# Meng-333/SRADSGAN

Measured on AMD Instinct MI355X. Metric: training images/sec (216x216, x4), higher is better.
Workload: dtype f32 (split-bf16 products: 3 bf16 MFMA terms per fp32 multiply, fp32 accumulate)

## Files before the change

include/sradsgan_hip.h:

```cpp
#ifndef SRADSGAN_HIP_H
#define SRADSGAN_HIP_H
#include <stddef.h>
#include <stdint.h>

#ifdef __cplusplus
extern "C" {
#endif

#define SRHIP_OK 0
#define SRHIP_ERR_ARG (-1)
#define SRHIP_ERR_LAUNCH (-2)
#define SRHIP_ERR_WORKSPACE (-3)

#define SRHIP_EPI_BIAS 1
#define SRHIP_EPI_LRELU 2
#define SRHIP_EPI_RESIDUAL 4
#define SRHIP_EPI_ROWSCALE 8
#define SRHIP_EPI_ACTMASK 32
#define SRHIP_EPI_CHANSCALE 16
#define SRHIP_EPI_GRADDATA 64

const char* srhip_last_error(void);
int srhip_abi_version(void);
int srhip_stream_fork(void* from_stream, void* to_stream);
// ... 197 lines not shown
int srhip_dp_init(const void* id_in, int rank, int world);
int srhip_dp_world(void);
int srhip_dp_rank(void);
int srhip_dp_allreduce_bucket(float* buf, size_t count, void* stream);
int srhip_dp_broadcast(float* buf, size_t count, int root, void* stream);
int srhip_dp_finalize(void);

size_t srhip_bn_workspace(long rows, int c);
int srhip_bn_train_fwd(const float* x, const float* gamma, const float* beta, float* running_mean,
                       float* running_var, float* y, float* save_mean, float* save_invstd, void* workspace,
                       size_t workspace_bytes, long rows, int c, float eps, float momentum, float slope, int apply_act,
                       void* stream);
int srhip_bn_train_bwd(const float* dy, const float* x, const float* y, const float* gamma, const float* save_mean,
                       const float* save_invstd, float* dx, float* dgamma, float* dbeta, void* workspace,
                       size_t workspace_bytes, long rows, int c, float slope, int apply_act, void* stream);
int srhip_bn_train_bwd_acc(const float* dy, const float* x, const float* y, const float* gamma, const float* save_mean,
                           const float* save_invstd, float* dx, float* dgamma, float* dbeta, float* acc_gamma,
                           float* acc_beta, void* workspace, size_t workspace_bytes, long rows, int c, float slope,
                           int apply_act, void* stream);
int srhip_bn_train_bwd_acc_x(const float* dy, const float* x, const float* gamma, const float* beta, const float* save_mean,
                             const float* save_invstd, float* dx, float* dgamma, float* dbeta, float* acc_gamma,
                             float* acc_beta, void* workspace, size_t workspace_bytes, long rows, int c, float slope,
                             int apply_act, void* stream);
int srhip_bn_train_bwd_acc_xa(const float* dy, const float* x, const float* gamma, const float* beta, const float* save_mean,
                              const float* save_invstd, const float* addend, float* dx, float* dgamma, float* dbeta, float* acc_gamma,
                              float* acc_beta, void* workspace, size_t workspace_bytes, long rows, int c, float slope,
                              int apply_act, void* stream);
int srhip_bn_eval_fwd(const float* x, const float* gamma, const float* beta, const float* running_mean,
                      const float* running_var, float* y, long rows, int c, float eps, float slope, int apply_act,
                      void* stream);
// ... 36 lines not shown
```

sradsgan_amd/_hip.py:

```python
import ctypes
import os

_HERE = os.path.dirname(os.path.abspath(__file__))
LIB_PATH = os.path.join(_HERE, 'lib', 'libsradsgan_hip.so')

_vp, _i, _f, _l, _sz = ctypes.c_void_p, ctypes.c_int, ctypes.c_float, ctypes.c_long, ctypes.c_size_t

SIGNATURES = {
    'srhip_last_error': (ctypes.c_char_p, []),
    'srhip_abi_version': (_i, []),
    'srhip_stream_fork': (_i, [_vp, _vp]),
    'srhip_debug_set': (_i, [_i, _i]),
    'srhip_probe_config': (_i, [_i] * 7),
    'srhip_probe_read': (_i, [_vp, _vp, _i]),
    'srhip_set_conv_math': (_i, [_i]),
    'srhip_get_conv_math': (_i, []),
    'srhip_resample_ksize': (_i, [_i, _i, _i]),
    'srhip_resample_coeffs': (_i, [_i, _i, _i, _vp, _vp]),
    'srhip_resample_pass_u8': (_i, [_vp, _vp, _vp, _vp, _i, _i, _i, _i, _i, _i, _i, _vp]),
    'srhip_u8_to_float': (_i, [_vp, _vp, _l, _vp]),
    'srhip_packed_elems': (_sz, [_i] * 5),
    'srhip_pack_entry_bytes': (_i, []),
    'srhip_packed_is_fast': (_i, [_i] * 5),
    'srhip_pack_weights_batched': (_i, [_vp, _i, _vp]),
# ... 71 lines not shown
    'srhip_mean_bwd': (_i, [_vp] * 2 + [_l, _vp]),
    'srhip_gp_norm_penalty_fwd': (_i, [_vp] * 3 + [_sz, _l, _i, _vp]),
    'srhip_gp_norm_penalty_bwd': (_i, [_vp] * 3 + [_l, _i, _vp]),
    'srhip_bn_eval_fwd': (_i, [_vp] * 6 + [_l, _i, _f, _f, _i, _vp]),
    'srhip_dp_id_bytes': (_i, []),
    'srhip_dp_unique_id': (_i, [_vp]),
    'srhip_dp_init': (_i, [_vp, _i, _i]),
    'srhip_dp_world': (_i, []),
    'srhip_dp_rank': (_i, []),
    'srhip_dp_allreduce_bucket': (_i, [_vp, _sz, _vp]),
    'srhip_dp_broadcast': (_i, [_vp, _sz, _i, _vp]),
    'srhip_dp_finalize': (_i, []),
    'srhip_bn_workspace': (_sz, [_l, _i]),
    'srhip_bn_train_fwd': (_i, [_vp] * 9 + [_sz, _l, _i, _f, _f, _f, _i, _vp]),
    'srhip_bn_train_bwd': (_i, [_vp] * 10 + [_sz, _l, _i, _f, _i, _vp]),
    'srhip_bn_bwd2_workspace': (_sz, [_l, _i]),
    'srhip_bn_train_bwd_bwd': (_i, [_vp] * 11 + [_sz, _l, _i, _f, _i, _vp]),
    'srhip_clam_pool_segments': (_i, []),
    'srhip_clam_pool_max_segments': (_i, []),
    'srhip_clam_pool_partial': (_i, [_vp, _vp, _sz, _i, _i, _i, _i, _vp]),
    'srhip_conv2d_fwd_pool': (_i, [_vp, _vp, _vp, _vp, _vp, _sz, _vp] + [_i] * 8 + [_vp]),
    'srhip_attn_tail_fwd_pooled': (_i, [_vp, _vp, _sz, _i] + [_vp] * 10 + [_i] * 5 + [_vp]),
    'srhip_attn_tail_eval_pooled': (_i, [_vp, _vp, _vp, _sz, _i] + [_vp] * 6 + [_i] * 5 + [_vp]),
    'srhip_sum_n': (_i, [_vp, _i, _vp, _l, _vp]),
    'srhip_ca_segments': (_i, []),
    'srhip_ca_pool_sum': (_i, [_vp, _vp] + [_i] * 3 + [_vp]),
    'srhip_ca_mlp_fwd': (_i, [_vp, _i] + [_vp] * 5 + [_i] * 4 + [_vp]),
    'srhip_ca_scale_res': (_i, [_vp] * 4 + [_i] * 3 + [_vp]),
    'srhip_ca_bwd_partial': (_i, [_vp] * 3 + [_i] * 3 + [_vp]),
    'srhip_ca_mlp_bwd_workspace': (_sz, [_i, _i]),
# ... 61 lines not shown
```

sradsgan_amd/csrc/bn.hip:

```cpp
#include "common.h"

namespace srhip {

__device__ inline float4 f4add(float4 a, float4 b) { return make_float4(a.x + b.x, a.y + b.y, a.z + b.z, a.w + b.w); }

template <int MODE>
__global__ __launch_bounds__(256) void bn_reduce_stage1(const float* __restrict__ a, const float* __restrict__ x,
                                                        const float* __restrict__ y, const float* __restrict__ mean,
                                                        const float* __restrict__ invstd, float* __restrict__ partial,
                                                        long rows, int c, long rows_per_block, float slope, int act,
                                                        const float* __restrict__ gamma = nullptr, const float* __restrict__ beta = nullptr) {
  __shared__ float4 red0[256], red1[256];
  const int tid = threadIdx.x;
  const int q = c / 4, nrl = 256 / q;
  const int cq = tid % q, rl = tid / q;
  const long r0 = (long)blockIdx.x * rows_per_block;
  const long r1 = r0 + rows_per_block < rows ? r0 + rows_per_block : rows;
  float4 s0 = make_float4(0.f, 0.f, 0.f, 0.f), s1 = s0;
  float4 p0, p1;
  if (MODE == 0) {
    p0 = *reinterpret_cast<const float4*>(x + cq * 4);
  } else {
    p0 = *reinterpret_cast<const float4*>(mean + cq * 4);
    p1 = *reinterpret_cast<const float4*>(invstd + cq * 4);
// ... 75 lines not shown
    const float n = (float)rows;
    const float md = s1 / n;
    float var = s2 / n - md * md;
    var = var > 0.f ? var : 0.f;
    const float mu = x[col] + md;
    mean[col] = mu;
    invstd[col] = rsqrtf(var + eps);
    if (running_mean) {
      running_mean[col] = (1.f - momentum) * running_mean[col] + momentum * mu;
      const float unb = rows > 1 ? var * (n / (n - 1.f)) : var;
      running_var[col] = (1.f - momentum) * running_var[col] + momentum * unb;
    }
  }
}

__global__ void bn_bwd_stage2(const float* __restrict__ partial, float* __restrict__ dgamma, float* __restrict__ dbeta,
                              int nblk, int c, float* __restrict__ acc_gamma, float* __restrict__ acc_beta) {
  __shared__ float r0[16 * BN_SUBS], r1[16 * BN_SUBS];
  const int col = blockIdx.x * 16 + (threadIdx.x & 15), sub = threadIdx.x >> 4;
  float a = 0.f, b = 0.f;
  if (col < c)
    for (int k = sub; k < nblk; k += BN_SUBS) {
      a += partial[(size_t)k * 2 * c + col];
      b += partial[(size_t)k * 2 * c + c + col];
    }
  r0[threadIdx.x] = a;
  r1[threadIdx.x] = b;
  __syncthreads();
  if (sub == 0 && col < c) {
    const int t = threadIdx.x;
// ... 271 lines not shown
  hipStream_t st = as_stream(stream);
  const long nblk = bn_nblk(rows), rpb = (rows + nblk - 1) / nblk;
  float* part = static_cast<float*>(workspace);
  hipLaunchKernelGGL(bn_reduce_stage1<0>, dim3((int)nblk), dim3(256), 0, st, nullptr, x, nullptr, nullptr, nullptr, part,
                     rows, c, rpb, 0.f, 0);
  hipLaunchKernelGGL(bn_stats_stage2, dim3(cdiv(c, 16)), dim3(16 * BN_SUBS), 0, st, part, x, save_mean, save_invstd, running_mean,
                     running_var, (int)nblk, c, rows, eps, momentum);
  const long n4 = rows * c / 4;
  int blocks = (int)((n4 + 255) / 256);
  if (blocks > 256 * 16) blocks = 256 * 16;
  hipLaunchKernelGGL(bn_apply_kernel, dim3(blocks), dim3(256), 0, st, x, save_mean, save_invstd, gamma, beta, y, n4, c,
                     slope, apply_act);
  return check_launch("bn_train_fwd");
}

int srhip_bn_eval_fwd(const float* x, const float* gamma, const float* beta, const float* running_mean,
                      const float* running_var, float* y, long rows, int c, float eps, float slope, int apply_act,
                      void* stream) {
  SRHIP_REQUIRE(x && gamma && beta && running_mean && running_var && y, "bn_eval_fwd: null tensor");
  SRHIP_REQUIRE(rows > 0 && c >= 4 && c % 4 == 0, "bn_eval_fwd: C must be a multiple of 4");
  const long n4 = rows * c / 4;
  int blocks = (int)((n4 + 255) / 256);
  if (blocks > 256 * 16) blocks = 256 * 16;
  hipLaunchKernelGGL(bn_eval_kernel, dim3(blocks), dim3(256), 0, as_stream(stream), x, running_mean, running_var, gamma, beta, y,
                     n4, c, eps, slope, apply_act);
  return check_launch("bn_eval_fwd");
}

int srhip_bn_train_bwd(const float* dy, const float* x, const float* y, const float* gamma, const float* save_mean,
                       const float* save_invstd, float* dx, float* dgamma, float* dbeta, void* workspace,
// ... 109 lines not shown
```

sradsgan_amd/csrc/conv_api.hip:

```cpp
#include "conv_internal.h"
#include "conv_dev.h"

using namespace srhip;

namespace srhip {
struct PackEntry {
  const float* w;
  float* packed;
  int cout, cin, kh, kw, mode, fast;
};
__global__ __launch_bounds__(256) void pack_batched_kernel(const PackEntry* __restrict__ tab) {
  const PackEntry e = tab[blockIdx.y];
  const int khkw = e.kh * e.kw;
  if (e.fast) {
    constexpr int LDS_F = 32 * (16 * 9 + 1);
    __shared__ float tile[LDS_F];
    const long total = (long)e.cout * e.cin * khkw;
    const int RO = e.mode == 0 ? 8 : 32;
    const int CI = e.mode == 0 ? (khkw <= 9 ? 64 : 16) : (khkw <= 9 ? 16 : 4);
    const int ld = CI * khkw + 1;
    const int nci = (e.cin + CI - 1) / CI, nco = (e.cout + RO - 1) / RO;
    const int ndst = e.mode == 0 ? e.cout : e.cin, csrc = e.mode == 0 ? e.cin : e.cout;
    const long ndst16 = ((long)ndst + 15) / 16 * 16;
    float* s0 = e.packed;
// ... 291 lines not shown

int srhip_conv2d_fwd_dual(const float* x, const float* packed, const float* bias, const float* residual, const float* rowscale,
                          const float* chanscale, float* y, void* y_pp, int* served, int n, int h, int w, int cin, int cout, int kh,
                          int kw, int stride, int pad, int ldx, int ldy, int ldr, float slope, int flags, void* stream) {
  SRHIP_REQUIRE(y_pp && served && (((uintptr_t)y_pp) & 15) == 0 && ldy == cout, "conv2d_fwd_dual: 16-byte aligned plane buffer, dense fp32 output");
  g_dst2_req.pp = y_pp;
  g_dst2_req.served = 0;
  const int rc = srhip_conv2d_fwd(x, packed, bias, residual, rowscale, chanscale, y, n, h, w, cin, cout, kh, kw, stride, pad, ldx, ldy, ldr,
                                  slope, flags, stream);
  *served = g_dst2_req.served;
  g_dst2_req.pp = nullptr;
  g_dst2_req.served = 0;
  return rc;
}

int srhip_conv2d_fwd_pool(const float* x, const float* packed, const float* bias, float* y, float* pool, size_t pool_sec_bytes,
                          int* nseg_out, int n, int h, int w, int cin, int cout, int ldx, int ldy, int flags, void* stream) {
  SRHIP_REQUIRE(x && packed && y && pool && nseg_out, "conv2d_fwd_pool: null tensor");
  SRHIP_REQUIRE(cout == 64 && ldy == 64 && n > 0 && h > 0 && w > 0 && cin > 0 && ldx >= cin, "conv2d_fwd_pool: 64 dense destination channels");
  SRHIP_REQUIRE((flags & ~SRHIP_EPI_BIAS) == 0 && (!(flags & SRHIP_EPI_BIAS) || bias), "conv2d_fwd_pool: plain or bias epilogue");
  SRHIP_REQUIRE(pool_sec_bytes % 16 == 0 && pool_sec_bytes < (1u << 30) && (((uintptr_t)pool) & 15) == 0 &&
                    pool_sec_bytes >= (size_t)n * POOL_MAXSEG * 64 * sizeof(float),
                "conv2d_fwd_pool: three 16-byte aligned sections of n * max_segments * 64 floats");
  g_pool_req.out = pool;
  g_pool_req.sec_bytes = (unsigned)pool_sec_bytes;
  g_pool_req.served_nseg = 0;
  const int rc = srhip_conv2d_fwd(x, packed, bias, nullptr, nullptr, nullptr, y, n, h, w, cin, cout, 3, 3, 1, 1, ldx, ldy, 0, 0.f, flags, stream);
  const int served = g_pool_req.served_nseg;
  g_pool_req.out = nullptr;
  g_pool_req.served_nseg = 0;
// ... 266 lines not shown
```

sradsgan_amd/csrc/conv_dev.h:

```cpp
#pragma once
#include "conv_internal.h"

namespace srhip {

typedef unsigned int u32x4 __attribute__((ext_vector_type(4)));
typedef unsigned int u32x2 __attribute__((ext_vector_type(2)));
constexpr int FBK = 16;
constexpr int FLS = FBK + 4;
constexpr unsigned F_OOB = 0x80000000u;

struct FastGeom {
  int N, Hs, Ws, C, lds;
  int OH, OW, M;
  int ss;
  int TH, TW, dh0, dhs, dw0, dws;
  int kh0, khs, kw0, kws, KW;
  int Hd, Wd, dsd, ph, pw, ldd, K;
  int ldw, ldr;
  float slope;
  int flags, accumulate, dst_identity;
  unsigned src_bytes, w_bytes;
  int src_pp = 0, dst_pp = 0, src_guard = 0, dst_guard = 0;
  unsigned src_plane_bytes = 0, dst_plane_bytes = 0;
  void* dst2_pp = nullptr;
  int dst2_guard = 0;
  const float* res2 = nullptr;
  const float* res3 = nullptr;
};
struct ResRequest {
  const float* r2 = nullptr;
  const float* r3 = nullptr;
  int served = 0;
};
extern thread_local ResRequest g_res_req;
struct SignRequest {
  void* words = nullptr;
  size_t bytes = 0;
  int mode = 0;
  int served = 0;
};
extern thread_local SignRequest g_sign_req;
long pp_sign_tiles(int n, int h, int w, int cout);
struct PhaseSet {
// ... 134 lines not shown
```

sradsgan_amd/csrc/conv_fast.hip:

```cpp
#include "conv_dev.h"

namespace srhip {

int g_fast_ablate = 0;



template <int BM, int BN, int WM, int WN, int BK, int MATH = 0>
__global__ __launch_bounds__(WM* WN * 64) void fast_conv_kernel(const float* __restrict__ src,
                                                                 const float* __restrict__ wt,
                                                                 const float* __restrict__ bias,
                                                                 const float* __restrict__ residual,
                                                                 const float* __restrict__ rowscale,
                                                                 const float* __restrict__ chanscale,
                                                                 const float* __restrict__ actmask,
                                                                 float* __restrict__ dst, FastGeom g, int nblk_m,
                                                                 int nblk_n) {
  constexpr int NT = WM * WN * 64;
  constexpr int WTM = BM / WM, WTN = BN / WN;
  constexpr int TM = WTM / 32, TN = WTN / 32;
  constexpr int LS = BK + 4;
  constexpr int QPR = BK / 4;
  constexpr int RPP = NT / QPR;
  constexpr int AR = (BM + RPP - 1) / RPP, BR = (BN + RPP - 1) / RPP;
// ... 581 lines not shown
          const int nimg = mm / OHOW;
          const int rem = mm - nimg * OHOW;
          const int oh = rem / g.OW;
          const int ow = rem - oh * g.OW;
          dpix = ((size_t)nimg * g.Hd + (oh * g.dsd + g.ph)) * g.Wd + (ow * g.dsd + g.pw);
        }
        dpx[j] = (unsigned)dpix;
        if (!okq[j]) nq[j] = 0;
        eo[j] = epi_fetch(dpix, nq[j], flags, g, bias, residual, rowscale, actmask, dst, EPI < 0 && g.accumulate != 0);
      }
#pragma unroll
      for (int j = 0; j < EB; ++j)
        if (okq[j]) epi_finish(vq[j], eo[j], dpx[j], nq[j], flags, g, dst, EPI < 0 && g.accumulate != 0);
    }
    if (t + 1 < TM) asm volatile("s_waitcnt lgkmcnt(0)" ::: "memory");
  }
}


template <int BN, int EPI, int PROD = 0>
__global__ __launch_bounds__(256) __attribute__((amdgpu_waves_per_eu(3))) void conv_patch_kernel(const float* __restrict__ src, const float* __restrict__ wt,
                                                          const float* __restrict__ bias,
                                                          const float* __restrict__ residual,
                                                          const float* __restrict__ actmask, float* __restrict__ dst,
                                                          FastGeom g, PatchGeom pg, int nblk_m, int nblk_n) {
  constexpr int NW = 4, BK = 16;
  constexpr int WTM = 64, WTN = BN / 2;
  constexpr int TM = WTM / 32, TN = WTN / 32;
  constexpr int BPW = BN / 64;
  constexpr int MAXP = 3;
// ... 1595 lines not shown
  }
}

static bool shape_ok(int csrc, int kh, int kw) { return csrc % 16 == 0 && kh * kw <= 32 && kh == kw; }
bool fast_fwd_ok(int cin, int cout, int kh, int kw) { return shape_ok(cin, kh, kw); }
bool fast_dgrad_ok(int cin, int cout, int kh, int kw) { return shape_ok(cout, kh, kw); }
bool fast_wgrad_ok(int cin, int cout, int kh, int kw) { return cin % 16 == 0 && cout % 4 == 0 && kh == kw; }

int fast_pack_weight(const float* w, float* packed, int cout, int cin, int kh, int kw, int mode, hipStream_t st) {
  const long total = (long)cout * cin * kh * kw;
  hipLaunchKernelGGL(fast_pack_kernel, dim3(cdiv(total, 256)), dim3(256), 0, st, w, packed, cout, cin, kh, kw, mode);
  return check_launch("fast_pack_weight");
}

thread_local Dst2Request g_dst2_req;
thread_local ResRequest g_res_req;
thread_local PhaseRequest g_phase_req;
int g_conv_math = 0;
int g_fast_dynlds = 0;
template <int BM, int BN, int WM, int WN, int BK>
static int launch_fast(const float* src, const float* wt, const float* bias, const float* residual,
                       const float* rowscale, const float* chanscale, const float* actmask, float* dst,
                       const FastGeom& g, hipStream_t st) {
  const int nbm = cdiv(g.M, BM), nbn = cdiv(g.K, BN);
  hipLaunchKernelGGL((fast_conv_kernel<BM, BN, WM, WN, BK>), dim3(nbm * nbn), dim3(WM * WN * 64), g_fast_dynlds, st, src, wt, bias,
                     residual, rowscale, chanscale, actmask, dst, g, nbm, nbn);
  return check_launch("fast_conv");
}

__global__ __launch_bounds__(256) void dot_conv_kernel(const float* __restrict__ src, const float* __restrict__ wt,
// ... 221 lines not shown
#undef SRHIP_LK
        }
        SRHIP_LPE(64);
#undef SRHIP_LPE
#undef SRHIP_LP
      }
    }
  }
  if (g_fast_cfg != 20 && (g_fast_cfg < 1 || g_fast_cfg == 23 || g_fast_cfg == 24) && !(g.flags & 0x300) && g.K >= 64 && al16 &&
      (!(eflags & SRHIP_EPI_CHANSCALE) || ((uintptr_t)chanscale & 15) == 0)) {
    const int nbm = cdiv(g.M, 128);
    const bool force = g_fast_cfg == -1 || patch_to_dma;
    const long min_tiles = g_conv_math >= 1 ? 128 : 512;
    const bool wide = g.K >= 128 && ((long)nbm * cdiv(g.K, 128) >= min_tiles || force);
    const long b64 = (long)nbm * cdiv(g.K, 64);
    if (wide || b64 >= min_tiles || force) {
#define SRHIP_LD(BN_, EPI_)                                                                                        \
  do {                                                                                                             \
    const int nbn = cdiv(g.K, BN_);                                                                                \
    if (g.dst2_pp) g_dst2_req.served = 1;                                                                          \
    PhaseSet ps_;                                                                                                  \
    int grid_ = nbm * nbn;                                                                                         \
    if (g_phase_req.active) {                            \
      ps_ = g_phase_req.ps;                                                                                        \
      grid_ = 0;                                                                                                   \
      for (int k_ = 0; k_ < ps_.n; ++k_) {                                                                         \
        ps_.first[k_] = grid_;                                                                                     \
        grid_ += ps_.p[k_].nblk_m * nbn;                                                                           \
      }                                                                                                            \
      ps_.first[ps_.n] = grid_;                                                                                    \
      g_phase_req.launched = 1;                                                                                    \
    }                                                                                                              \
    if (g_conv_math == 1) {                                                                                        \
      hipLaunchKernelGGL((fast_conv_dma_kernel<128, BN_, EPI_, 1>), dim3(grid_), dim3(256), g_fast_dynlds, st,     \
                         src, w16, bias, residual, rowscale, chanscale, actmask, dst, g, nbm,                      \
                         nbn, ps_);                                                                                \
    } else                                                                                                         \
      hipLaunchKernelGGL((fast_conv_dma_kernel<128, BN_, EPI_, 0>), dim3(grid_), dim3(256), g_fast_dynlds, st,     \
                         src, wt, bias, residual, rowscale, chanscale, actmask, dst, g, nbm, nbn, ps_);            \
    return check_launch("fast_conv_dma");                                                                          \
  } while (0)
#define SRHIP_LDE(BN_)                                                  \
  do {                                                                  \
    if (g.accumulate) SRHIP_LD(BN_, -1);                                \
    if (eflags == 0) SRHIP_LD(BN_, 0);                                  \
    if (eflags == SRHIP_EPI_BIAS) SRHIP_LD(BN_, 1);                     \
    if (eflags == (SRHIP_EPI_BIAS | SRHIP_EPI_LRELU)) SRHIP_LD(BN_, 3); \
    if (eflags == SRHIP_EPI_ACTMASK) SRHIP_LD(BN_, 32);                 \
    if (eflags == SRHIP_EPI_RESIDUAL) SRHIP_LD(BN_, 4);                 \
    if (eflags == 29) SRHIP_LD(BN_, 29);  \
    SRHIP_LD(BN_, -1);                                                  \
  } while (0)
      if (prod != 0) {
#define SRHIP_LDH(BN_, MATH_)                                                                                       \
  do {                                                                                                              \
    const int nbn = cdiv(g.K, BN_);                                                                                 \
    hipLaunchKernelGGL((fast_conv_dma_kernel<128, BN_, -1, MATH_>), dim3(nbm * nbn), dim3(256), g_fast_dynlds, st,  \
                       src, w16, bias, residual, rowscale, chanscale, actmask, dst, g, nbm, nbn, PhaseSet());       \
// ... 45 lines not shown
  g.OW = (w + 2 * pad - kw) / stride + 1;
  SRHIP_REQUIRE(g.OH > 0 && g.OW > 0, "conv2d_fwd: empty output");
  const long M = (long)n * g.OH * g.OW;
  SRHIP_REQUIRE(M < (1L << 31), "conv2d_fwd: pixel count overflows int32");
  g.M = (int)M; g.ss = stride;
  g.TH = kh; g.TW = kw; g.dh0 = -pad; g.dhs = 1; g.dw0 = -pad; g.dws = 1;
  g.kh0 = 0; g.khs = 1; g.kw0 = 0; g.kws = 1; g.KW = kw;
  g.Hd = g.OH; g.Wd = g.OW; g.dsd = 1; g.ph = 0; g.pw = 0; g.ldd = ldy; g.K = cout;
  g.ldw = kh * kw * cin; g.ldr = ldr; g.slope = slope; g.flags = flags | g_fast_ablate; g.accumulate = 0; g.dst_identity = 1;
  SRHIP_REQUIRE(bytes_ok((long)n * h * w, ldx, cin, &g.src_bytes), "conv2d_fwd: source tensor >= 2 GiB");
  g.w_bytes = (unsigned)((long)cout * g.ldw * 4);
  if (g_dst2_req.pp != nullptr && stride == 1 && cout % 8 == 0 && g.OH == g.Hd && g.OW == g.Wd) {
    g.dst2_pp = g_dst2_req.pp;
    g.dst2_guard = pp_guard(g.Wd);
  }
  return run_fast(x, packed, bias, residual, rowscale, chanscale, nullptr, y, g, st);
}

int fast_conv2d_fwd_pp(const void* x, int x_pp, const float* packed, const float* bias, void* y, int y_pp, int n, int h, int w, int cin,
                       int cout, int ldx, int ldy, float slope, int flags, hipStream_t st) {
  FastGeom g;
  g.N = n; g.Hs = h; g.Ws = w; g.C = cin; g.lds = x_pp ? cin : ldx;
  g.OH = h; g.OW = w;
  const long M = (long)n * h * w;
  SRHIP_REQUIRE(M < (1L << 31), "conv2d_fwd_pp: pixel count overflows int32");
  g.M = (int)M; g.ss = 1;
  g.TH = 3; g.TW = 3; g.dh0 = -1; g.dhs = 1; g.dw0 = -1; g.dws = 1;
  g.kh0 = 0; g.khs = 1; g.kw0 = 0; g.kws = 1; g.KW = 3;
  g.Hd = h; g.Wd = w; g.dsd = 1; g.ph = 0; g.pw = 0; g.ldd = y_pp ? cout : ldy; g.K = cout;
  g.ldw = 9 * cin; g.ldr = 0; g.slope = slope; g.flags = flags; g.accumulate = 0; g.dst_identity = 1;
// ... 404 lines not shown
```

sradsgan_amd/csrc/elementwise.hip:

```cpp
#include <atomic>
#include <mutex>
#include "conv_internal.h"

#include <string.h>

namespace srhip {

static thread_local char g_err[512] = "";

void set_error(const char* fmt, ...) {
  va_list ap;
  va_start(ap, fmt);
  vsnprintf(g_err, sizeof(g_err), fmt, ap);
  va_end(ap);
}

__global__ void lrelu_bwd_kernel(const float4* __restrict__ dy, const float4* __restrict__ y, float4* __restrict__ dx,
                                 long n4, float slope) {
  long i = (long)blockIdx.x * blockDim.x + threadIdx.x;
  long stride = (long)gridDim.x * blockDim.x;
  for (; i < n4; i += stride) {
    float4 g = dy[i], v = y[i];
    g.x = v.x > 0.f ? g.x : g.x * slope;
    g.y = v.y > 0.f ? g.y : g.y * slope;
// ... 370 lines not shown
  if (vec)
    hipLaunchKernelGGL(colsum_stage1<float4>, dim3((int)nblk), dim3(256), 0, st, dy, (float*)workspace, rows, c, ld, rpb);
  else
    hipLaunchKernelGGL(colsum_stage1<float>, dim3((int)nblk), dim3(256), 0, st, dy, (float*)workspace, rows, c, ld, rpb);
  hipLaunchKernelGGL(colsum_stage2, dim3(cdiv(c, 16)), dim3(256), 0, st, (const float*)workspace, db, (int)nblk, c);
  return check_launch("colsum");
}

}

using namespace srhip;

extern "C" {

const char* srhip_last_error(void) { return g_err; }
int srhip_abi_version(void) { return 13; }

int srhip_stream_fork(void* from_stream, void* to_stream) {
  constexpr int RING = 64;
  static hipEvent_t ring[RING];
  static std::atomic<unsigned> next{0};
  static std::once_flag once;
  static bool created = false;
  if (from_stream == to_stream) return SRHIP_OK;
  std::call_once(once, [&]() {
    created = true;
    for (int i = 0; i < RING; ++i)
      if (hipEventCreateWithFlags(&ring[i], hipEventDisableTiming) != hipSuccess) created = false;
  });
  if (!created) {
    set_error("stream_fork: hipEventCreateWithFlags failed");
// ... 190 lines not shown
```

sradsgan_amd/model/layers.py:

```python
import torch
import torch.nn as nn

from .. import ops


class HipConv2d(nn.Conv2d):

    def __init__(self, *args, **kwargs):
        super().__init__(*args, **kwargs)
        k, s, p, d = self.kernel_size, self.stride, self.padding, self.dilation
        if k[0] != k[1] or s[0] != s[1] or p[0] != p[1] or d != (1, 1) or self.groups != 1:
            raise NotImplementedError('HipConv2d: square kernel/stride/pad, dilation 1, groups 1 only')

    def forward(self, x, act_slope=None, residual=None):
        return ops.conv2d(x, self.weight, self.bias, self.stride[0], self.padding[0], act_slope, residual)


class HipBatchNorm2d(nn.BatchNorm2d):

    def forward(self, x, act_slope=None):
        return ops.batch_norm_act(x, self, act_slope)
```

sradsgan_amd/model/sradsgan.py:

```python
import math

import torch
import torch.nn as nn

from .. import ops
from .base_networks import ChannelAttention, SpatialAttention, _Clam, _Slam
from .layers import HipBatchNorm2d, HipConv2d


class GANLoss(nn.Module):

    def __init__(self, gan_type, real_label_val=1.0, fake_label_val=0.0):
        super().__init__()
        self.gan_type = gan_type.lower()
        self.real_label_val, self.fake_label_val = real_label_val, fake_label_val
        if self.gan_type != 'wgan-gp':
            raise NotImplementedError('GAN type [{:s}] is not found'.format(self.gan_type))

    def forward(self, input, target_is_real):
        m = ops.mean(input)
        return -m if target_is_real else m


class CLAM(_Clam):
# ... 232 lines not shown
            if attention and idx == 6:
                entry[2] = [len(layers), len(layers) + 1]
                layers += [ChannelAttention(256), SpatialAttention()]
            self._blocks.append(tuple(entry))
            cin = cout
        layers.append(HipConv2d(cin, 1, 3, 1, 1))
        self.model = nn.Sequential(*layers)

    def forward(self, img):
        x = ops.nhwc(img)
        m = self.model
        for conv_i, bn_i, extra in self._blocks:
            if bn_i is None:
                x = m[conv_i](x, act_slope=0.2)
            else:
                x = m[bn_i](m[conv_i](x), act_slope=0.2)
            for e in extra:
                x = m[e](x)
        return m[len(m) - 1](x)


class FeatureExtractor(nn.Module):

    _CFG = [(3, 64), 'R', (64, 64), 'R', 'P', (64, 128), 'R', (128, 128), 'R', 'P', (128, 256), 'R']

    def __init__(self):
        super().__init__()
        seq = []
        for item in self._CFG:
            seq.append(HipConv2d(item[0], item[1], 3, 1, 1) if isinstance(item, tuple) else nn.Identity())
        self.feature_extractor = nn.Sequential(*seq)
# ... 23 lines not shown
```

sradsgan_amd/ops.py:

```python
import contextlib
import ctypes
import os
import threading
import weakref

import torch
from torch.autograd import Function

from . import _hip

EPI_BIAS, EPI_LRELU, EPI_RESIDUAL, EPI_ROWSCALE, EPI_CHANSCALE, EPI_GRADDATA = 1, 2, 4, 8, 16, 64
CL = torch.channels_last

class _State:
    skip_param_grads = False
    direct_grads = False
    wgrad_stream = None
    skip_ids = frozenset()
    stop_ids = frozenset()
    capturing = False
    wgrad_group = 1
    pending = None
    held = None
    last_out_pp = None
    carry = None
    carry_expect = None
    carry_token = 0
    wgrad_seq = 0
    ready_pairs = None


_state = _State()


def _skip_param_grads(*params):
    if _state.skip_param_grads:
        return True
    return bool(_state.skip_ids) and any(p is not None and id(p) in _state.skip_ids for p in params)


@contextlib.contextmanager
def backward_scope(skip_params=(), stop_at=()):
    prev = (_state.skip_ids, _state.stop_ids)
    _state.skip_ids = frozenset(id(p) for p in skip_params)
# ... 289 lines not shown
    lib = _hip.lib()
    if out_pp is not None:
        served = ctypes.c_int(0)
        _hip.check(lib.srhip_conv2d_fwd_dual(_p(x), _p(packed_weight(w, 0)), _p(bias), _p(residual), _p(rowscale),
                                             _p(chanscale), _p(y), _p(out_pp.buf), ctypes.byref(served),
                                             n, h, wd, cin, cout, kh, kw, stride, pad, cin, cout, cout,
                                             float(slope or 0.0), flags, _stream()), 'conv2d_fwd_dual')
        if not served.value:
            pp_from_f32(y, out=out_pp)
        return y
    _hip.check(lib.srhip_conv2d_fwd(_p(x), _p(packed_weight(w, 0)), _p(bias), _p(residual), _p(rowscale),
                                    _p(chanscale), _p(y),
                                    n, h, wd, cin, cout, kh, kw, stride, pad, cin, cout, cout,
                                    float(slope or 0.0), flags, _stream()), 'conv2d_fwd')
    return y


_POOL_EPI = os.environ.get('SRHIP_POOL_EPI', '1') == '1'


def pool_epilogue_ok(x, w):
    return (_POOL_EPI and x.is_cuda and get_conv_math() == 'bf16x3' and tuple(w.shape[2:]) == (3, 3) and w.shape[0] == 64
            and w.shape[1] % 32 == 0)


def conv2d_fwd_pool_raw(x, w, bias):
    _require_gpu(x, 'conv2d_fwd_pool')
    x = nhwc(x)
    n, cin, h, wd = x.shape
    cout = w.shape[0]
# ... 619 lines not shown

class _ColSum(Function):
    @staticmethod
    def forward(ctx, dy):
        ctx.shape = dy.shape
        return colsum_raw(dy)

    @staticmethod
    def backward(ctx, g):
        return g.view(1, -1, 1, 1).expand(ctx.shape)


class _ConvFwd(Function):

    @staticmethod
    def forward(ctx, x, w, b, residual, stride, pad, slope, graddata=False):
        if slope is not None and residual is not None:
            raise ValueError('conv2d: fused activation and residual are mutually exclusive')
        y = conv2d_fwd_raw(x, w, b, stride, pad, slope, residual, graddata=graddata)
        ctx.stride, ctx.pad, ctx.slope = stride, pad, slope
        ctx.has_bias, ctx.has_res = b is not None, residual is not None
        ctx.save_for_backward(x, w, y if slope is not None else None, b)
        return y

    @staticmethod
    def backward(ctx, dy):
        x, w, y, b = ctx.saved_tensors
        skip = _skip_param_grads(w)
        need_dx = ctx.needs_input_grad[0] and x.data_ptr() not in _state.stop_ids
        if ctx.slope is not None and not need_dx and not skip and ctx.needs_input_grad[1] and ctx.has_bias and \
                ctx.needs_input_grad[2] and _state.direct_grads and not torch.is_grad_enabled() and _WGRAD_ACT and \
                _wgrad_act_direct(w, b, x, dy, y, ctx.slope, ctx.stride, ctx.pad):
            return None, None, None, None, None, None, None, None
        g = dy if ctx.slope is None else _LReluBwd.apply(dy, y, ctx.slope)
        dx = _ConvDgrad.apply(g, w, tuple(x.shape), ctx.stride, ctx.pad) if need_dx else None
        dw = db = None
        want_b = ctx.has_bias and ctx.needs_input_grad[2] and not skip
        if ctx.needs_input_grad[1] and not skip and _state.direct_grads and not torch.is_grad_enabled():
            dw, db = wgrad_for_params(w, b, x, g, ctx.stride, ctx.pad, want_b)
        elif ctx.needs_input_grad[1] and not skip:
            dw, db = _ConvWgrad.apply(x, g, tuple(w.shape), ctx.stride, ctx.pad, want_b)
        elif want_b:
            db = _ColSum.apply(g)
        dres = _passed_through(dy) if (ctx.has_res and ctx.needs_input_grad[3]) else None
        return dx, dw, db, dres, None, None, None, None


class _ConvDgrad(Function):

    @staticmethod
    def forward(ctx, dy, w, x_shape, stride, pad):
        ctx.stride, ctx.pad, ctx.x_shape = stride, pad, x_shape
        ctx.save_for_backward(dy, w)
        return conv2d_dgrad_raw(dy, w, x_shape, stride, pad)

    @staticmethod
    def backward(ctx, ddx):
        dy, w = ctx.saved_tensors
        skip = _skip_param_grads(w)
        d_dy = _ConvFwd.apply(ddx, w, None, None, ctx.stride, ctx.pad, None, True) if ctx.needs_input_grad[0] else None
# ... 20 lines not shown
    def backward(ctx, ddw, ddb):
        x, dy = ctx.saved_tensors
        d_x = d_dy = None
        if ddw is not None:
            ddw = ddw.contiguous()
            if ctx.needs_input_grad[0]:
                d_x = _ConvDgrad.apply(dy, ddw, tuple(x.shape), ctx.stride, ctx.pad)
            if ctx.needs_input_grad[1]:
                d_dy = _ConvFwd.apply(x, ddw, None, None, ctx.stride, ctx.pad, None, True)
        if ddb is not None and ctx.needs_input_grad[1]:
            e = ddb.view(1, -1, 1, 1).expand(dy.shape)
            d_dy = e if d_dy is None else d_dy + e
        return d_x, d_dy, None, None, None, None


def conv2d(x, weight, bias=None, stride=1, padding=0, act_slope=None, residual=None):
    return _ConvFwd.apply(x, weight, bias, residual, stride, padding, act_slope)


_BUS_SUM = os.environ.get('SRHIP_BUS_SUM', '1') == '1'


class _SumN(Function):

    @staticmethod
    def forward(ctx, tokens, *ts):
        _require_gpu(ts[0], 'sum_n')
        ts = [nhwc(t) for t in ts]
        out = torch.empty_like(ts[0], memory_format=CL)
        tab = (ctypes.c_void_p * len(ts))(*[t.data_ptr() for t in ts])
        _hip.check(_hip.lib().srhip_sum_n(tab, len(ts), _p(out), out.numel(), _stream()), 'sum_n')
        ctx.n, ctx.tokens = len(ts), tokens
# ... 760 lines not shown
            gdy, gx, gg = torch.autograd.grad([o for o, _ in pairs], [dy_, x_, g_], [d for _, d in pairs],
                                              allow_unused=True)
        return gdy, gx, None, gg, None, None, None, None, None, None, None, None


class _BNTrainFwd(Function):
    @staticmethod
    def forward(ctx, x, gamma, beta, running_mean, running_var, eps, momentum, slope):
        _require_gpu(x, 'batch_norm')
        xc = nhwc(x)
        n, c, h, w = x.shape
        rows = n * h * w
        lib = _hip.lib()
        y = torch.empty_like(xc, memory_format=CL)
        mean, invstd = torch.empty_like(gamma), torch.empty_like(gamma)
        ws = torch.empty(lib.srhip_bn_workspace(rows, c) // 4, device=x.device, dtype=torch.float32)
        _hip.check(lib.srhip_bn_train_fwd(_p(xc), _p(gamma.detach().contiguous()), _p(beta.detach().contiguous()),
                                          _p(running_mean), _p(running_var), _p(y), _p(mean), _p(invstd), _p(ws),
                                          ws.numel() * 4, rows, c, float(eps), float(momentum), float(slope or 0.0),
                                          int(slope is not None), _stream()), 'bn_train_fwd')
        ctx.eps, ctx.slope = eps, slope
        ctx.save_for_backward(x, y, gamma, mean, invstd, beta)
        return y

    @staticmethod
    def backward(ctx, dy):
        x, y, gamma, mean, invstd, beta = ctx.saved_tensors
        fold = getattr(_state, 'bn_fold', None)
        held = fold.pop((x.data_ptr(), tuple(x.shape)), None) if (fold and not torch.is_grad_enabled()) else None
        if not torch.is_grad_enabled() and not _skip_param_grads(gamma, beta):
            gg, gb = _grad_slot(gamma), _grad_slot(beta)
            if gg is not None and gb is not None:
                dx, _, _ = _BNTrainBwd.apply(dy, x, y, gamma, mean, invstd, ctx.eps, ctx.slope, gg, gb, beta, held)
                return dx, None, None, None, None, None, None, None
        dx, dgamma, dbeta = _BNTrainBwd.apply(dy, x, y, gamma, mean, invstd, ctx.eps, ctx.slope, None, None, beta, held)
# ... 719 lines not shown
```

Baseline: 665.4.

## Fuse BatchNorm batch-statistics reduction into conv forward epilogue

Adds a conv epilogue variant that computes per-wave, per-channel mean and M2 partials straight from the accumulators and writes them to a slot buffer. A new merge kernel combines these slots Chan-style into mean and invstd and updates the running stats, then the existing apply kernel runs. This skips the separate BN stage-1 reduction pass over the conv output in the discriminator's conv+BN blocks. It costs extra epilogue shuffles and registers in the conv kernel, relies on thread-local handoff state and Python-side pointer/version matching, and the pairwise merge may be slightly less numerically stable.

After: 665.0 (median of 6 runs). Within noise of the previous version (-0.0%).

```diff
diff --git a/include/sradsgan_hip.h b/include/sradsgan_hip.h
--- a/include/sradsgan_hip.h
+++ b/include/sradsgan_hip.h
@@ -235,6 +235,13 @@
 int srhip_bn_train_bwd(const float* dy, const float* x, const float* y, const float* gamma, const float* save_mean,
                        const float* save_invstd, float* dx, float* dgamma, float* dbeta, void* workspace,
                        size_t workspace_bytes, long rows, int c, float slope, int apply_act, void* stream);
+size_t srhip_conv2d_bnstat_bytes(int n, int h, int w, int cout, int kh, int kw, int stride, int pad);
+int srhip_conv2d_fwd_bnstat(const float* x, const float* packed, const float* bias, float* y, float* partial, size_t partial_bytes,
+                            int* nslot_out, int* slot_rows_out, int n, int h, int w, int cin, int cout, int kh, int kw, int stride,
+                            int pad, int flags, void* stream);
+int srhip_bn_train_fwd_merged(const float* partial, int nslot, int slot_rows, const float* x, const float* gamma, const float* beta,
+                              float* running_mean, float* running_var, float* y, float* save_mean, float* save_invstd, long rows, int c,
+                              float eps, float momentum, float slope, int apply_act, void* stream);
 int srhip_bn_train_bwd_acc(const float* dy, const float* x, const float* y, const float* gamma, const float* save_mean,
                            const float* save_invstd, float* dx, float* dgamma, float* dbeta, float* acc_gamma,
                            float* acc_beta, void* workspace, size_t workspace_bytes, long rows, int c, float slope,
diff --git a/sradsgan_amd/_hip.py b/sradsgan_amd/_hip.py
--- a/sradsgan_amd/_hip.py
+++ b/sradsgan_amd/_hip.py
@@ -109,6 +109,9 @@
     'srhip_bn_workspace': (_sz, [_l, _i]),
     'srhip_bn_train_fwd': (_i, [_vp] * 9 + [_sz, _l, _i, _f, _f, _f, _i, _vp]),
     'srhip_bn_train_bwd': (_i, [_vp] * 10 + [_sz, _l, _i, _f, _i, _vp]),
+    'srhip_conv2d_bnstat_bytes': (_sz, [_i] * 8),
+    'srhip_conv2d_fwd_bnstat': (_i, [_vp] * 5 + [_sz, _vp, _vp] + [_i] * 10 + [_vp]),
+    'srhip_bn_train_fwd_merged': (_i, [_vp, _i, _i] + [_vp] * 8 + [_l, _i, _f, _f, _f, _i, _vp]),
     'srhip_bn_bwd2_workspace': (_sz, [_l, _i]),
     'srhip_bn_train_bwd_bwd': (_i, [_vp] * 11 + [_sz, _l, _i, _f, _i, _vp]),
     'srhip_clam_pool_segments': (_i, []),
diff --git a/sradsgan_amd/csrc/bn.hip b/sradsgan_amd/csrc/bn.hip
--- a/sradsgan_amd/csrc/bn.hip
+++ b/sradsgan_amd/csrc/bn.hip
@@ -113,6 +113,54 @@
   }
 }
 
+__global__ void bn_stats_merge(const float* __restrict__ partial, int nslot, int slot_rows, float* __restrict__ mean,
+                               float* __restrict__ invstd, float* __restrict__ running_mean, float* __restrict__ running_var, int c,
+                               long rows, float eps, float momentum) {
+  __shared__ float r0[16 * BN_SUBS], r1[16 * BN_SUBS], r2[16 * BN_SUBS], r3[16 * BN_SUBS];
+  const int col = blockIdx.x * 16 + (threadIdx.x & 15), sub = threadIdx.x >> 4;
+  float s0 = 0.f, s1 = 0.f, s2 = 0.f, sq = 0.f;
+  const float K = col < c ? partial[col] : 0.f;
+  if (col < c) {
+    const long full = rows / slot_rows;
+#pragma unroll 4
+    for (int k = sub; k < nslot; k += BN_SUBS) {
+      const float nb = k < full ? (float)slot_rows : (float)(k == full ? rows - full * slot_rows : 0);
+      const float d = partial[(size_t)k * 2 * c + col] - K;
+      const float q = partial[(size_t)k * 2 * c + c + col];
+      s0 += nb;
+      s1 += nb * d;
+      s2 += nb * d * d;
+      sq += nb > 0.f ? q : 0.f;
+    }
+  }
+  r0[threadIdx.x] = s0;
+  r1[threadIdx.x] = s1;
+  r2[threadIdx.x] = s2;
+  r3[threadIdx.x] = sq;
+  __syncthreads();
+  if (sub == 0 && col < c) {
+    const int t = threadIdx.x;
+    for (int k = 1; k < BN_SUBS; ++k) {
+      s0 += r0[t + 16 * k];
+      s1 += r1[t + 16 * k];
+      s2 += r2[t + 16 * k];
+      sq += r3[t + 16 * k];
+    }
+    const float nr = (float)rows;
+    const float md = s1 / s0;
+    float var = (sq + (s2 - s1 * md)) / nr;
+    var = var > 0.f ? var : 0.f;
+    const float mu = K + md;
+    mean[col] = mu;
+    invstd[col] = rsqrtf(var + eps);
+    if (running_mean) {
+      running_mean[col] = (1.f - momentum) * running_mean[col] + momentum * mu;
+      const float unb = rows > 1 ? var * (nr / (nr - 1.f)) : var;
+      running_var[col] = (1.f - momentum) * running_var[col] + momentum * unb;
+    }
+  }
+}
+
 __global__ void bn_bwd_stage2(const float* __restrict__ partial, float* __restrict__ dgamma, float* __restrict__ dbeta,
                               int nblk, int c, float* __restrict__ acc_gamma, float* __restrict__ acc_beta) {
   __shared__ float r0[16 * BN_SUBS], r1[16 * BN_SUBS];
@@ -414,6 +462,24 @@
   return check_launch("bn_train_fwd");
 }
 
+int srhip_bn_train_fwd_merged(const float* partial, int nslot, int slot_rows, const float* x, const float* gamma, const float* beta,
+                              float* running_mean, float* running_var, float* y, float* save_mean, float* save_invstd, long rows, int c,
+                              float eps, float momentum, float slope, int apply_act, void* stream) {
+  SRHIP_REQUIRE(partial && x && gamma && beta && y && save_mean && save_invstd, "bn_train_fwd_merged: null tensor");
+  SRHIP_REQUIRE(rows > 0 && c >= 4 && c % 4 == 0, "bn_train_fwd_merged: C must be a multiple of 4");
+  SRHIP_REQUIRE(nslot > 0 && slot_rows > 0 && (long)nslot * slot_rows >= rows, "bn_train_fwd_merged: the slots do not cover the rows");
+  SRHIP_REQUIRE((running_mean == nullptr) == (running_var == nullptr), "bn_train_fwd_merged: running stats come in pairs");
+  hipStream_t st = as_stream(stream);
+  hipLaunchKernelGGL(bn_stats_merge, dim3(cdiv(c, 16)), dim3(16 * BN_SUBS), 0, st, partial, nslot, slot_rows, save_mean, save_invstd,
+                     running_mean, running_var, c, rows, eps, momentum);
+  const long n4 = rows * c / 4;
+  int blocks = (int)((n4 + 255) / 256);
+  if (blocks > 256 * 16) blocks = 256 * 16;
+  hipLaunchKernelGGL(bn_apply_kernel, dim3(blocks), dim3(256), 0, st, x, save_mean, save_invstd, gamma, beta, y, n4, c,
+                     slope, apply_act);
+  return check_launch("bn_train_fwd_merged");
+}
+
 int srhip_bn_eval_fwd(const float* x, const float* gamma, const float* beta, const float* running_mean,
                       const float* running_var, float* y, long rows, int c, float eps, float slope, int apply_act,
                       void* stream) {
diff --git a/sradsgan_amd/csrc/conv_api.hip b/sradsgan_amd/csrc/conv_api.hip
--- a/sradsgan_amd/csrc/conv_api.hip
+++ b/sradsgan_amd/csrc/conv_api.hip
@@ -329,6 +329,37 @@
   return rc;
 }
 
+size_t srhip_conv2d_bnstat_bytes(int n, int h, int w, int cout, int kh, int kw, int stride, int pad) {
+  if (n <= 0 || h <= 0 || w <= 0 || cout <= 0 || kh <= 0 || kw <= 0 || stride <= 0 || pad < 0) return 0;
+  const long oh = (h + 2 * pad - kh) / stride + 1, ow = (w + 2 * pad - kw) / stride + 1;
+  if (oh <= 0 || ow <= 0) return 0;
+  const long slots = cdiv(n * oh * ow, 2L * BNSTAT_ROWS) * 2;
+  return (size_t)slots * 2 * cout * sizeof(float);
+}
+int srhip_conv2d_fwd_bnstat(const float* x, const float* packed, const float* bias, float* y, float* partial, size_t partial_bytes,
+                            int* nslot_out, int* slot_rows_out, int n, int h, int w, int cin, int cout, int kh, int kw, int stride,
+                            int pad, int flags, void* stream) {
+  SRHIP_REQUIRE(x && packed && y && partial && nslot_out && slot_rows_out, "conv2d_fwd_bnstat: null tensor");
+  SRHIP_REQUIRE((flags & ~SRHIP_EPI_BIAS) == 0 && (!(flags & SRHIP_EPI_BIAS) || bias), "conv2d_fwd_bnstat: plain or bias epilogue");
+  const size_t need = srhip_conv2d_bnstat_bytes(n, h, w, cout, kh, kw, stride, pad);
+  SRHIP_REQUIRE(need > 0 && partial_bytes >= need && (((uintptr_t)partial) & 15) == 0, "conv2d_fwd_bnstat: partial buffer too small");
+  *nslot_out = 0;
+  *slot_rows_out = BNSTAT_ROWS;
+  const bool fast = fast_fwd_ok(cin, cout, kh, kw);
+  if (fast) {
+    g_bnstat_req.out = partial;
+    g_bnstat_req.served = 0;
+  }
+  const int rc = srhip_conv2d_fwd(x, packed, bias, nullptr, nullptr, nullptr, y, n, h, w, cin, cout, kh, kw, stride, pad, cin, cout, 0, 0.f,
+                                  flags, stream);
+  const int served = fast ? g_bnstat_req.served : 0;
+  g_bnstat_req.out = nullptr;
+  g_bnstat_req.served = 0;
+  if (rc != SRHIP_OK) return rc;
+  if (served) *nslot_out = (int)(need / (2 * cout * sizeof(float)));
+  return SRHIP_OK;
+}
+
 int srhip_conv2d_fwd_pool(const float* x, const float* packed, const float* bias, float* y, float* pool, size_t pool_sec_bytes,
                           int* nseg_out, int n, int h, int w, int cin, int cout, int ldx, int ldy, int flags, void* stream) {
   SRHIP_REQUIRE(x && packed && y && pool && nseg_out, "conv2d_fwd_pool: null tensor");
diff --git a/sradsgan_amd/csrc/conv_dev.h b/sradsgan_amd/csrc/conv_dev.h
--- a/sradsgan_amd/csrc/conv_dev.h
+++ b/sradsgan_amd/csrc/conv_dev.h
@@ -26,7 +26,15 @@
   int dst2_guard = 0;
   const float* res2 = nullptr;
   const float* res3 = nullptr;
+  float* bnstat = nullptr;
 };
+constexpr int BNSTAT_EPI = 0x800;
+constexpr int BNSTAT_ROWS = 64;
+struct BnStatRequest {
+  float* out = nullptr;
+  int served = 0;
+};
+extern thread_local BnStatRequest g_bnstat_req;
 struct ResRequest {
   const float* r2 = nullptr;
   const float* r3 = nullptr;
diff --git a/sradsgan_amd/csrc/conv_fast.hip b/sradsgan_amd/csrc/conv_fast.hip
--- a/sradsgan_amd/csrc/conv_fast.hip
+++ b/sradsgan_amd/csrc/conv_fast.hip
@@ -619,6 +619,53 @@
         if (okq[j]) epi_finish(vq[j], eo[j], dpx[j], nq[j], flags, g, dst, EPI < 0 && g.accumulate != 0);
     }
     if (t + 1 < TM) asm volatile("s_waitcnt lgkmcnt(0)" ::: "memory");
+  }
+  if constexpr (EPI >= 0 && (EPI & BNSTAT_EPI) != 0) {
+    static_assert(WTM == BNSTAT_ROWS, "one partial slot per wave's rows");
+#pragma unroll
+    for (int u = 0; u < TN; ++u) {
+      const int col = n0 + wn * WTN + u * 32 + l31;
+      const bool cok = col < g.K;
+      const float bb = ((EPI & SRHIP_EPI_BIAS) && cok) ? bias[col] : 0.f;
+      const float K = __shfl(acc[0][u][0] + bb, l31);
+      float cnt = 0.f, mu = 0.f, m2 = 0.f;
+#pragma unroll
+      for (int t = 0; t < TM; ++t) {
+        const int mrow = m0 + wm * WTM + t * 32 + 4 * khalf;
+        float s = 0.f, k = 0.f;
+#pragma unroll
+        for (int r = 0; r < 16; ++r)
+          if (mrow + (r & 3) + 8 * (r >> 2) < g.M) {
+            s += (acc[t][u][r] + bb) - K;
+            k += 1.f;
+          }
+        s += __shfl_xor(s, 32);
+        k += __shfl_xor(k, 32);
+        const float mt = k > 0.f ? s / k : 0.f;
+        float q = 0.f;
+#pragma unroll
+        for (int r = 0; r < 16; ++r)
+          if (mrow + (r & 3) + 8 * (r >> 2) < g.M) {
+            const float d = ((acc[t][u][r] + bb) - K) - mt;
+            q += d * d;
+          }
+        q += __shfl_xor(q, 32);
+        if (t == 0 || cnt == 0.f) {
+          cnt = k; mu = mt; m2 = q;
+        } else if (k > 0.f) {
+          const float nn = cnt + k, d = mt - mu;
+          mu += d * (k / nn);
+          m2 += q + d * d * (cnt * k / nn);
+          cnt = nn;
+        }
+      }
+      mu += K;
+      if (khalf == 0 && cok) {
+        float* o = g.bnstat + (size_t)(tile_m * WM + wm) * 2 * g.K + col;
+        o[0] = mu;
+        o[g.K] = m2;
+      }
+    }
   }
 }
 
@@ -2244,6 +2291,7 @@
 }
 
 thread_local Dst2Request g_dst2_req;
+thread_local BnStatRequest g_bnstat_req;
 thread_local ResRequest g_res_req;
 thread_local PhaseRequest g_phase_req;
 int g_conv_math = 0;
@@ -2495,11 +2543,14 @@
     const long min_tiles = g_conv_math >= 1 ? 128 : 512;
     const bool wide = g.K >= 128 && ((long)nbm * cdiv(g.K, 128) >= min_tiles || force);
     const long b64 = (long)nbm * cdiv(g.K, 64);
+    const bool bnst = g.bnstat != nullptr && !g.accumulate && !g_phase_req.active && g.dst_identity && !g.dst2_pp && !patch_to_dma &&
+                      (eflags == 0 || eflags == SRHIP_EPI_BIAS);
     if (wide || b64 >= min_tiles || force) {
 #define SRHIP_LD(BN_, EPI_)                                                                                        \
   do {                                                                                                             \
     const int nbn = cdiv(g.K, BN_);                                                                                \
     if (g.dst2_pp) g_dst2_req.served = 1;                                                                          \
+    if ((EPI_) >= 0 && ((EPI_) & BNSTAT_EPI)) g_bnstat_req.served = 1;                                            \
     PhaseSet ps_;                                                                                                  \
     int grid_ = nbm * nbn;                                                                                         \
     if (g_phase_req.active) {                            \
@@ -2523,6 +2574,8 @@
   } while (0)
 #define SRHIP_LDE(BN_)                                                  \
   do {                                                                  \
+    if (bnst && eflags == 0) SRHIP_LD(BN_, BNSTAT_EPI);                 \
+    if (bnst && eflags == SRHIP_EPI_BIAS) SRHIP_LD(BN_, BNSTAT_EPI | SRHIP_EPI_BIAS); \
     if (g.accumulate) SRHIP_LD(BN_, -1);                                \
     if (eflags == 0) SRHIP_LD(BN_, 0);                                  \
     if (eflags == SRHIP_EPI_BIAS) SRHIP_LD(BN_, 1);                     \
@@ -2598,6 +2651,7 @@
     g.dst2_pp = g_dst2_req.pp;
     g.dst2_guard = pp_guard(g.Wd);
   }
+  g.bnstat = g_bnstat_req.out;
   return run_fast(x, packed, bias, residual, rowscale, chanscale, nullptr, y, g, st);
 }
 
diff --git a/sradsgan_amd/csrc/elementwise.hip b/sradsgan_amd/csrc/elementwise.hip
--- a/sradsgan_amd/csrc/elementwise.hip
+++ b/sradsgan_amd/csrc/elementwise.hip
@@ -408,7 +408,7 @@
 extern "C" {
 
 const char* srhip_last_error(void) { return g_err; }
-int srhip_abi_version(void) { return 13; }
+int srhip_abi_version(void) { return 14; }
 
 int srhip_stream_fork(void* from_stream, void* to_stream) {
   constexpr int RING = 64;
diff --git a/sradsgan_amd/model/layers.py b/sradsgan_amd/model/layers.py
--- a/sradsgan_amd/model/layers.py
+++ b/sradsgan_amd/model/layers.py
@@ -12,8 +12,8 @@
         if k[0] != k[1] or s[0] != s[1] or p[0] != p[1] or d != (1, 1) or self.groups != 1:
             raise NotImplementedError('HipConv2d: square kernel/stride/pad, dilation 1, groups 1 only')
 
-    def forward(self, x, act_slope=None, residual=None):
-        return ops.conv2d(x, self.weight, self.bias, self.stride[0], self.padding[0], act_slope, residual)
+    def forward(self, x, act_slope=None, residual=None, bn_stats=False):
+        return ops.conv2d(x, self.weight, self.bias, self.stride[0], self.padding[0], act_slope, residual, bn_stats)
 
 
 class HipBatchNorm2d(nn.BatchNorm2d):
diff --git a/sradsgan_amd/model/sradsgan.py b/sradsgan_amd/model/sradsgan.py
--- a/sradsgan_amd/model/sradsgan.py
+++ b/sradsgan_amd/model/sradsgan.py
@@ -270,7 +270,7 @@
             if bn_i is None:
                 x = m[conv_i](x, act_slope=0.2)
             else:
-                x = m[bn_i](m[conv_i](x), act_slope=0.2)
+                x = m[bn_i](m[conv_i](x, bn_stats=True), act_slope=0.2)
             for e in extra:
                 x = m[e](x)
         return m[len(m) - 1](x)
diff --git a/sradsgan_amd/ops.py b/sradsgan_amd/ops.py
--- a/sradsgan_amd/ops.py
+++ b/sradsgan_amd/ops.py
@@ -28,6 +28,7 @@
     carry_token = 0
     wgrad_seq = 0
     ready_pairs = None
+    bn_partials = None
 
 
 _state = _State()
@@ -347,6 +348,38 @@
                                     n, h, wd, cin, cout, kh, kw, stride, pad, cin, cout, cout,
                                     float(slope or 0.0), flags, _stream()), 'conv2d_fwd')
     return y
+
+
+_BN_CONV_STATS = os.environ.get('SRHIP_BN_CONV_STATS', '1') == '1'
+
+
+def conv2d_fwd_bnstat_raw(x, w, bias, stride, pad):
+    _require_gpu(x, 'conv2d_fwd_bnstat')
+    x = nhwc(x)
+    n, cin, h, wd = x.shape
+    cout, _, kh, kw = w.shape
+    ho, wo = _out_hw(h, wd, kh, stride, pad)
+    y = empty_nhwc(n, cout, ho, wo, x)
+    lib = _hip.lib()
+    nbytes = lib.srhip_conv2d_bnstat_bytes(n, h, wd, cout, kh, kw, stride, pad)
+    part = torch.empty(max(nbytes // 4, 4), device=x.device, dtype=torch.float32)
+    nslot, rows = ctypes.c_int(0), ctypes.c_int(0)
+    b = bias.detach().contiguous() if bias is not None else None
+    _hip.check(lib.srhip_conv2d_fwd_bnstat(_p(x), _p(packed_weight(w, 0)), _p(b), _p(y), _p(part), part.numel() * 4, ctypes.byref(nslot),
+                                           ctypes.byref(rows), n, h, wd, cin, cout, kh, kw, stride, pad, EPI_BIAS if b is not None else 0,
+                                           _stream()), 'conv2d_fwd_bnstat')
+    return y, ((part, nslot.value, rows.value) if nslot.value > 0 else None)
+
+
+def _bn_partials_put(y, part):
+    _state.bn_partials = (y, y._version, part[0], part[1], part[2])
+
+
+def _bn_partials_take(x):
+    ent, _state.bn_partials = _state.bn_partials, None
+    if ent is None or ent[0].data_ptr() != x.data_ptr() or ent[0].shape != x.shape or ent[1] != x._version:
+        return None
+    return ent[2:]
 
 
 _POOL_EPI = os.environ.get('SRHIP_POOL_EPI', '1') == '1'
@@ -996,10 +1029,15 @@
 class _ConvFwd(Function):
 
     @staticmethod
-    def forward(ctx, x, w, b, residual, stride, pad, slope, graddata=False):
+    def forward(ctx, x, w, b, residual, stride, pad, slope, graddata=False, bn_stats=False):
         if slope is not None and residual is not None:
             raise ValueError('conv2d: fused activation and residual are mutually exclusive')
-        y = conv2d_fwd_raw(x, w, b, stride, pad, slope, residual, graddata=graddata)
+        if bn_stats and _BN_CONV_STATS and slope is None and residual is None and not graddata and x.is_cuda:
+            y, part = conv2d_fwd_bnstat_raw(x, w, b, stride, pad)
+            if part is not None:
+                _bn_partials_put(y, part)
+        else:
+            y = conv2d_fwd_raw(x, w, b, stride, pad, slope, residual, graddata=graddata)
         ctx.stride, ctx.pad, ctx.slope = stride, pad, slope
         ctx.has_bias, ctx.has_res = b is not None, residual is not None
         ctx.save_for_backward(x, w, y if slope is not None else None, b)
@@ -1013,7 +1051,7 @@
         if ctx.slope is not None and not need_dx and not skip and ctx.needs_input_grad[1] and ctx.has_bias and \
                 ctx.needs_input_grad[2] and _state.direct_grads and not torch.is_grad_enabled() and _WGRAD_ACT and \
                 _wgrad_act_direct(w, b, x, dy, y, ctx.slope, ctx.stride, ctx.pad):
-            return None, None, None, None, None, None, None, None
+            return None, None, None, None, None, None, None, None, None
         g = dy if ctx.slope is None else _LReluBwd.apply(dy, y, ctx.slope)
         dx = _ConvDgrad.apply(g, w, tuple(x.shape), ctx.stride, ctx.pad) if need_dx else None
         dw = db = None
@@ -1025,7 +1063,7 @@
         elif want_b:
             db = _ColSum.apply(g)
         dres = _passed_through(dy) if (ctx.has_res and ctx.needs_input_grad[3]) else None
-        return dx, dw, db, dres, None, None, None, None
+        return dx, dw, db, dres, None, None, None, None, None
 
 
 class _ConvDgrad(Function):
@@ -1076,8 +1114,8 @@
         return d_x, d_dy, None, None, None, None
 
 
-def conv2d(x, weight, bias=None, stride=1, padding=0, act_slope=None, residual=None):
-    return _ConvFwd.apply(x, weight, bias, residual, stride, padding, act_slope)
+def conv2d(x, weight, bias=None, stride=1, padding=0, act_slope=None, residual=None, bn_stats=False):
+    return _ConvFwd.apply(x, weight, bias, residual, stride, padding, act_slope, False, bn_stats)
 
 
 _BUS_SUM = os.environ.get('SRHIP_BUS_SUM', '1') == '1'
@@ -1868,11 +1906,18 @@
         lib = _hip.lib()
         y = torch.empty_like(xc, memory_format=CL)
         mean, invstd = torch.empty_like(gamma), torch.empty_like(gamma)
-        ws = torch.empty(lib.srhip_bn_workspace(rows, c) // 4, device=x.device, dtype=torch.float32)
-        _hip.check(lib.srhip_bn_train_fwd(_p(xc), _p(gamma.detach().contiguous()), _p(beta.detach().contiguous()),
-                                          _p(running_mean), _p(running_var), _p(y), _p(mean), _p(invstd), _p(ws),
-                                          ws.numel() * 4, rows, c, float(eps), float(momentum), float(slope or 0.0),
-                                          int(slope is not None), _stream()), 'bn_train_fwd')
+        part = _bn_partials_take(xc)
+        if part is not None:
+            _hip.check(lib.srhip_bn_train_fwd_merged(_p(part[0]), part[1], part[2], _p(xc), _p(gamma.detach().contiguous()),
+                                                     _p(beta.detach().contiguous()), _p(running_mean), _p(running_var), _p(y), _p(mean),
+                                                     _p(invstd), rows, c, float(eps), float(momentum), float(slope or 0.0),
+                                                     int(slope is not None), _stream()), 'bn_train_fwd_merged')
+        else:
+            ws = torch.empty(lib.srhip_bn_workspace(rows, c) // 4, device=x.device, dtype=torch.float32)
+            _hip.check(lib.srhip_bn_train_fwd(_p(xc), _p(gamma.detach().contiguous()), _p(beta.detach().contiguous()),
+                                              _p(running_mean), _p(running_var), _p(y), _p(mean), _p(invstd), _p(ws),
+                                              ws.numel() * 4, rows, c, float(eps), float(momentum), float(slope or 0.0),
+                                              int(slope is not None), _stream()), 'bn_train_fwd')
         ctx.eps, ctx.slope = eps, slope
         ctx.save_for_backward(x, y, gamma, mean, invstd, beta)
         return y
```
